# josiahbjorgaard/mca-paper

Measured on AMD Instinct MI355X. Metric: training samples/sec (fwd+bwd+opt), CMU 4-modality MCA, higher is better.
Workload: dtype bf16; 1 GPU; synthetic CMU 4-modality (MCA fcl), N=2538 D=512 L=5 H=8 F=88, lengths=full, p_drop=0.0; per_gpu_batch=32, global_batch=32, parallelism=dp1, inputs=device-resident, same batch every step, finite_checks=on (device flag, polled), attention_operands=bf16, attention_backward=bf16 one-pass, launch=hipGraph replay (one launch per step), collectives=none

## Files before the change

### include/mca_hip.h

```cpp
#ifndef MCA_HIP_H
#define MCA_HIP_H
#include <stdint.h>

#ifdef __cplusplus
extern "C" {
#endif

typedef void* mca_stream_t;

#define MCA_OK 0
#define MCA_E_BADARG (-1)
#define MCA_E_ALIGN (-2)
#define MCA_E_UNSUPPORTED (-3)
#define MCA_E_LAUNCH (-4)

const char* mca_version(void);

int mca_gemm_nt(const uint16_t* A, int64_t lda, const uint16_t* B, int64_t ldb,
                void* C, int64_t ldc, int out_bf16,
                const float* bias, const float* residual, int64_t ldres, int64_t res_period,
                int64_t M, int64_t N, int64_t K, mca_stream_t stream);

int mca_gemm_nt_lnres(const uint16_t* A, int64_t lda, const uint16_t* B, int64_t ldb, float* C, int64_t ldc,
                      const float* x, int64_t ldx, const float* mean, const float* rstd, const float* gamma,
                      int64_t M, int64_t N, int64_t K, mca_stream_t stream);

int mca_gemm_nt_geglu_bwd(const uint16_t* A, int64_t lda, const uint16_t* B, int64_t ldb, const uint16_t* h,
                          uint16_t* dh, int64_t ldh, int64_t ip, int64_t M, int64_t K, mca_stream_t stream);

int mca_gemm_nt_geglu_fwd(const uint16_t* A, int64_t lda, const uint16_t* W1, int64_t ldb, uint16_t* h, int64_t ldh,
                          uint16_t* g, int64_t ldg, int64_t ip, int64_t M, int64_t K, mca_stream_t stream);

int mca_gemm_tn_acc(const uint16_t* A, int64_t lda, const uint16_t* B, int64_t ldb,
                    float* C, int64_t ldc, int64_t R, int64_t N, int64_t K, mca_stream_t stream);

#define MCA_TN_MAX_GROUP 8
typedef struct mca_tn_desc {
  const uint16_t* A; int64_t lda;
  const uint16_t* B; int64_t ldb;
  float* C; int64_t ldc;
  int64_t N, K;
} mca_tn_desc;
int mca_gemm_tn_acc_group(const mca_tn_desc* d, int n, int64_t R, mca_stream_t stream);

int mca_layernorm_fwd(const float* x, int64_t ldx, const float* gamma, const float* beta,
                      const uint8_t* rowmask, const float* add, int64_t period,
                      float* y, int64_t ldy, int64_t y_bstride,
                      uint16_t* y_bf16, int64_t ld_bf16, int cols_pad,
                      float* mean, float* rstd, int64_t rows, int cols, float eps, mca_stream_t stream);

int mca_layernorm_bwd(const float* dy, int64_t ldy, int64_t y_bstride, int64_t period,
                      const float* x, int64_t ldx, const float* gamma,
                      const float* mean, const float* rstd, const uint8_t* rowmask,
                      float* dx, int64_t lddx, uint16_t* dx_bf16, int64_t ld_bf16,
                      float* dgamma, float* dbeta, float* dxsum, int64_t rows, int cols, mca_stream_t stream);

int mca_geglu_fwd(const uint16_t* h, uint16_t* g, int64_t rows, int ip, mca_stream_t stream);
// ... 163 lines not shown
```

### mca-paper_amd/csrc/gemm.hip

```cpp
#include "common.h"

#define g_knob mca_knobs

#define BM 128
#define BN 128
#define BK 64

static int num_cus() {
  static int n = 0;
  if (!n) {
    int dev = 0;
    if (hipGetDevice(&dev) != hipSuccess || hipDeviceGetAttribute(&n, hipDeviceAttributeMultiprocessorCount, dev) != hipSuccess || n <= 0) n = 256;
  }
  return n;
}

#define PS_PANELS 4
__device__ __forceinline__ void ps_tile_decode(int tile, int tiles_m, int tiles_n, int flat, int& tm, int& tn) {
  if (flat == 1) { tm = tile / tiles_n; tn = tile % tiles_n; return; }
  const int P = flat > 1 ? flat : PS_PANELS;
  const int per_group = P * tiles_n;
  const int g = tile / per_group;
  const int gh = (g + 1) * P <= tiles_m ? P : tiles_m - g * P;
  const int rem = tile - g * per_group;
// ... 790 lines not shown
        u16* cp = C + (int64_t)m * ldc + nw + 8 * (lane & 15);
        if (m < M) PS_GSTORE(cp, o[u]);
      }
      if (GEGLU) {
        asm volatile("s_waitcnt lgkmcnt(0)\n\ts_barrier" ::: "memory");
        const unsigned sa = lds_base + 3u * (unsigned)(P2_STAGE * 2) + (unsigned)(wave & ~1) * 8192u, sg = sa + 8192u;
        u32x4v av[4], gv[4];
#pragma unroll
        for (int u = 0; u < 4; u++) {
          const int row = 16 * wn + (lane >> 4) + 4 * u, ch = lane & 15;
          NT_DSREAD(av[u], sa + (unsigned)(row * 256 + ((ch ^ (row & 15)) << 4)));
          NT_DSREAD(gv[u], sg + (unsigned)(row * 256 + ((ch ^ (row & 15)) << 4)));
        }
        asm volatile("s_waitcnt lgkmcnt(0)" ::: "memory");
#pragma unroll
        for (int u = 0; u < 4; u++) {
          const int m = m0 + wm * 64 + i * 32 + 16 * wn + (lane >> 4) + 4 * u;
          u32x4v gg;
#pragma unroll
          for (int e = 0; e < 4; e++) {
            const float a0 = __uint_as_float(av[u][e] << 16), a1 = __uint_as_float(av[u][e] & 0xffff0000u);
            const float g0 = __uint_as_float(gv[u][e] << 16), g1 = __uint_as_float(gv[u][e] & 0xffff0000u);
            float ge0, ge1, unused;
            gelu_pair(g0, ge0, unused); gelu_pair(g1, ge1, unused);
            gg[e] = pack2bf(a0 * ge0, a1 * ge1);
          }
          u16* gp = G + (int64_t)m * ldg + tn * 128 + 8 * (lane & 15);
          if (m < M) PS_GSTORE(gp, gg);
        }
        if (i == 0) asm volatile("s_barrier" ::: "memory");
      }
    }
    if (edge) ps_wait_vm<0>();
    first = false;
    v = vn;
  }
}

extern "C" int mca_gemm_nt(const uint16_t* A, int64_t lda, const uint16_t* B, int64_t ldb, void* C, int64_t ldc,
                           int out_bf16, const float* bias, const float* residual, int64_t ldres,
                           int64_t res_period, int64_t M, int64_t N, int64_t K, mca_stream_t stream) {
  if (!A || !B || !C || M <= 0 || N <= 0 || K <= 0) return MCA_E_BADARG;
  if (K % 64 || lda % 8 || ldb % 8 || (uintptr_t)A % 16 || (uintptr_t)B % 16) return MCA_E_ALIGN;
  if (lda < K || ldb < K || ldc < N) return MCA_E_BADARG;
  if (M > (1LL << 30) || N > (1LL << 30)) return MCA_E_UNSUPPORTED;
  const int tiles_m = (int)((M + BM - 1) / BM), tiles_n = (int)((N + BN - 1) / BN);
  const int nwg = tiles_m * tiles_n;
  const int res = !residual ? 0 : (res_period > 0 ? 2 : 1);
  const bool big = M >= 2048 && g_knob[1] != 1;
  const int nwg2 = (int)((M + BM2 - 1) / BM2) * tiles_n;
#define NT_LAUNCH_G(OB, RS)                                                                                              \
  hipLaunchKernelGGL((gemm_nt_glds_kernel<OB, RS, 64, 0>), dim3(nwg), dim3(256), 0, as_stream(stream), A, lda, B, ldb, C,   \
                     ldc, bias, residual, ldres, res_period, (int)M, (int)N, (int)K, tiles_n, nwg)
#define NT_LAUNCH_256(OB, RS, PFV)                                                                                          \
  do {                                                                                                                   \
    static bool attr_dev[64] = {false}; bool& attr = *mca_dev_flag(attr_dev);                                                                                            \
    if (!attr) {                                                                                                         \
      if (hipFuncSetAttribute(reinterpret_cast<const void*>(gemm_nt_256_kernel<OB, RS, PFV, 0>),                            \
                              hipFuncAttributeMaxDynamicSharedMemorySize, NT256_LDS_BYTES) != hipSuccess)                \
        return MCA_E_LAUNCH;                                                                                             \
      attr = true;                                                                                                       \
    }                                                                                                                    \
    hipLaunchKernelGGL((gemm_nt_256_kernel<OB, RS, PFV, 0>), dim3(nwg2), dim3(512), NT256_LDS_BYTES, as_stream(stream), A, lda, \
                       B, ldb, C, ldc, bias, residual, ldres, res_period, (int)M, (int)N, (int)K, tiles_n, nwg2);        \
  } while (0)
#define NT_PICK_PF(OB, RS) do { if (big) NT_LAUNCH_256(OB, RS, 0); else NT_LAUNCH_G(OB, RS); } while (0)
// ... 31 lines not shown
    else if (res == 0) { if (bias) NT_LAUNCH_PS(1, true); else NT_LAUNCH_PS(1, false); }
    else { if (bias) NT_LAUNCH_PS(2, true); else NT_LAUNCH_PS(2, false); }
    return launch_status();
  }
  const bool pf = big && !out_bf16 && res == 1 && N % BN == 0 && K >= 512 && ldres % 4 == 0 && ldc % 4 == 0 &&
                  (uintptr_t)residual % 16 == 0 && (uintptr_t)C % 16 == 0 && (!bias || (uintptr_t)bias % 4 == 0) && g_knob[4] != 1;
  if (pf) { NT_LAUNCH_256(false, 1, 1); return launch_status(); }
  if (out_bf16) { if (res == 0) NT_PICK_PF(true, 0); else if (res == 1) NT_PICK_PF(true, 1); else NT_PICK_PF(true, 2); }
  else { if (res == 0) NT_PICK_PF(false, 0); else if (res == 1) NT_PICK_PF(false, 1); else NT_PICK_PF(false, 2); }
  return launch_status();
}


extern "C" int mca_gemm_nt_lnres(const uint16_t* A, int64_t lda, const uint16_t* B, int64_t ldb, float* C, int64_t ldc,
                                 const float* x, int64_t ldx, const float* mean, const float* rstd, const float* gamma,
                                 int64_t M, int64_t N, int64_t K, mca_stream_t stream) {
  if (!A || !B || !C || !x || !mean || !rstd || !gamma || M <= 0 || N <= 0 || K <= 0) return MCA_E_BADARG;
  if (K % 64 || lda % 8 || ldb % 8 || ldc % 4 || ldx % 4 || (uintptr_t)A % 16 || (uintptr_t)B % 16 || (uintptr_t)C % 16 ||
      (uintptr_t)x % 16 || (uintptr_t)gamma % 16)
    return MCA_E_ALIGN;
  if (lda < K || ldb < K || ldc < N || ldx < N) return MCA_E_BADARG;
  if (M < 2048 || M > (1LL << 30) || N % BN || K < 512) return MCA_E_UNSUPPORTED;
  const int tiles_n = (int)(N / BN);
  const int nwg2 = (int)((M + BM2 - 1) / BM2) * tiles_n;
  static bool attr_dev[64] = {false}; bool& attr = *mca_dev_flag(attr_dev);
  if (!attr) {
    if (hipFuncSetAttribute(reinterpret_cast<const void*>(gemm_nt_256_kernel<false, 1, 1, 2>), hipFuncAttributeMaxDynamicSharedMemorySize,
                            NT256LN_LDS_BYTES) != hipSuccess)
      return MCA_E_LAUNCH;
    attr = true;
  }
  hipLaunchKernelGGL((gemm_nt_256_kernel<false, 1, 1, 2>), dim3(nwg2), dim3(512), NT256LN_LDS_BYTES, as_stream(stream), A, lda, B, ldb,
                     (void*)C, ldc, (const float*)nullptr, x, ldx, (int64_t)0, (int)M, (int)N, (int)K, tiles_n, nwg2, mean, rstd, gamma);
  return launch_status();
}

extern "C" int mca_gemm_nt_geglu_bwd(const uint16_t* A, int64_t lda, const uint16_t* B, int64_t ldb, const uint16_t* h,
                                     uint16_t* dh, int64_t ldh, int64_t ip, int64_t M, int64_t K, mca_stream_t stream) {
  if (!A || !B || !h || !dh || M <= 0 || ip <= 0 || K <= 0) return MCA_E_BADARG;
  if (K % 64 || lda % 8 || ldb % 8 || ldh % 8 || ip % 8 || (uintptr_t)A % 16 || (uintptr_t)B % 16 || (uintptr_t)h % 16 || (uintptr_t)dh % 16)
    return MCA_E_ALIGN;
  if (lda < K || ldb < K || ldh < 2 * ip) return MCA_E_BADARG;
  if (M > (1LL << 30)) return MCA_E_UNSUPPORTED;
  const int64_t N = ip;
  const int tiles_n = (int)((N + BN - 1) / BN);
  const float* hres = reinterpret_cast<const float*>(h);
  void* C = dh;
  if (M >= 40960 && g_knob[1] != 1) {
    const int nwg2 = (int)((M + BM2 - 1) / BM2) * tiles_n;
    static bool attr_dev[64] = {false}; bool& attr = *mca_dev_flag(attr_dev);
    if (!attr) {
      if (hipFuncSetAttribute(reinterpret_cast<const void*>(gemm_nt_256_kernel<true, 0, 0, 1>), hipFuncAttributeMaxDynamicSharedMemorySize,
                              NT256_LDS_BYTES) != hipSuccess ||
          hipFuncSetAttribute(reinterpret_cast<const void*>(gemm_nt_persist_kernel<3, false>), hipFuncAttributeMaxDynamicSharedMemorySize,
                              NTPS_LDS_BYTES) != hipSuccess)
        return MCA_E_LAUNCH;
      attr = true;
    }
    if (g_knob[7] != 1 && N % BN == 0 && K >= 320) {
      const int grid = nwg2 < num_cus() ? nwg2 : num_cus();
      hipLaunchKernelGGL((gemm_nt_persist_kernel<3, false>), dim3(grid), dim3(512), NTPS_LDS_BYTES, as_stream(stream), A, lda, B, ldb, C, ldh,
                         nullptr, hres, ldh, (int)M, (int)N, (int)K, tiles_n, nwg2, g_knob[0]);
    } else
      hipLaunchKernelGGL((gemm_nt_256_kernel<true, 0, 0, 1>), dim3(nwg2), dim3(512), NT256_LDS_BYTES, as_stream(stream), A, lda, B, ldb, C,
                         ldh, nullptr, hres, ldh, 0, (int)M, (int)N, (int)K, tiles_n, nwg2);
  } else {
// ... 673 lines not shown
```

### mca-paper_amd/engine.py

```python
from __future__ import annotations

import os

import ctypes as C
import math
from typing import Callable, Dict, List, Optional

import numpy as np
import torch

from . import attention, hip
from .attention import AttnGrads, AttnOperands, _OnePassSched, _Sched, _dev
from .encoders import EmbeddedSequenceEncoder, TabularEncoder
from .hip import AttnBwd1Args, AttnBwd2Args, AttnFp8BwdOperands, AttnFp8Operands, AttnFwdArgs, LossTerm, call, ptr, stream_ptr

LN_EPS = 1e-5
FWD_BQ, FWD_BK = 128, 64
BWD_BQ = 64


def _pad_to(x: int, m: int) -> int:
    return (x + m - 1) // m * m


def debug_options() -> dict:
    opts = {"overlap_wgrad": None, "group_wgrad": True, "mask_mfma": True, "dkv_keys": 128, "lazy_softmax": True,
            "onepass": None}
    for item in filter(None, os.environ.get("MCA_DEBUG", "").split(",")):
        k, _, v = item.partition("=")
        k = k.strip()
        if k not in opts:
            raise ValueError(f"MCA_DEBUG: unknown switch '{k}' (known: {sorted(opts)})")
        opts[k] = int(v) if k == "dkv_keys" else (v.strip() not in ("0", "", "false"))
    return opts


class FusionEngine:
    def __init__(self, model):
        self.model = model
        p0 = next(model.parameters())
        self.eao = model.attn_pool is None
        if p0.device.type != "cuda":
            raise hip.MCAHipError("the MCA step runs only on a HIP device: move the model to cuda first "
                                  "(there is no CPU fallback)")
        hip.lib()
        self.device = p0.device
        self.D, self.H, self.L = model.dim, model.heads, model.depth
        st = model.structure
        self.st = st
        self.N, self.R, self.F, self.M = st.n_tokens, st.n_return, st.num_fusion_tokens, st.n_modalities
        if self.D != self.H * 64:
            raise NotImplementedError("native path needs dim == heads * 64")
        self.I = model.layers[0].ff.inner_dim if self.L else int(self.D * 4 * 2 / 3)
        self.Ip = _pad_to(self.I, 64)
        self.scale = model.dim_head ** -0.5
        self.q_scale = self.scale * 1.4426950408889634
        self.attn_flags = hip.ATTN_Q_PRESCALED
        self.attn_dtype = "bf16"
        self.dbg = debug_options()
        if self.dbg["lazy_softmax"]:
            self.attn_flags |= hip.ATTN_LAZY_REFERENCE
        self.nk_pad = _pad_to(self.N, 256)
        self.mask_mfma = int(self.st.kgroup.max()) <= 14 and self.dbg["mask_mfma"]
        self._flatten_parameters()
        self._build_static()
        self._alloc_weights()
        self._ws: Dict[int, dict] = {}
        self._weights_version = -1
        self.grad_bucket_hook: Optional[Callable[[int, int], None]] = None
        self.gather_hook: Optional[Callable] = None
        self.check_finite = True
        self.finite_flag = torch.zeros(1, dtype=torch.int32, device=self.device)
        self._flag_host = torch.zeros(1, dtype=torch.int32).pin_memory()
        self._flag_event: Optional[torch.cuda.Event] = None
        self.fuse_geglu_bwd = True
        self._mod_shifts = torch.arange(len(model.modality_types), dtype=torch.int32, device=self.device)
        self.fuse_ln_residual = True
        self.overlap_wgrad = self.dbg["overlap_wgrad"]
        self.group_wgrad = self.dbg["group_wgrad"]

    def _flatten_parameters(self):
        m = self.model
        order: List[torch.nn.Parameter] = []
        marks: List[int] = []
        order += [m.loss.loss_fn.logit_scale]
        pool_kv_late = not self.eao and self.L > 0
        if not self.eao:
            order += [m.return_tokens, m.attn_pool.to_out.weight, m.attn_pool.to_q.weight]
            if not pool_kv_late:
                order += [m.attn_pool.to_kv.weight]
        order += [m.norm.gamma]
        marks.append(len(order))
        if pool_kv_late:
            order += [m.attn_pool.to_kv.weight]
        for i in reversed(range(self.L)):
            ly = m.layers[i]
            order += [ly.ff.feedforward[2].weight, ly.ff.feedforward[0].weight, ly.attn.to_out.weight,
                      ly.attn.to_q.weight, ly.attn.to_kv.weight, ly.norm.gamma]
            marks.append(len(order))
        if not self.eao:
            order.append(m.fusion_tokens)
        for name in m.modality_types:
            order += list(m.encoders[name].parameters())
        marks.append(len(order))
        seen = {id(p) for p in order}
        for p in m.parameters():
            if id(p) not in seen:
                order.append(p)
        marks[-1] = len(order)
        offs, n = [], 0
# ... 207 lines not shown
        ws["dpool_b"], ws["dop"], ws["dqp32"], ws["dqp_sum"], ws["dqp_b"] = bf(b * R, D), bf(b * R, D), f32(b * R, D), f32(R, D), bf(R, D)
        ws["dkvp"], ws["drt"] = (None if self.eao else bf(T, 2 * D)), f32(R, D)
        sc = self.sched_onepass
        if sc is not None:
            rc = f32(b, H, sc.n_qt + 1, 2, 64)
            rc[:, :, :, 0] = float("-inf"); rc[:, :, :, 1] = 0.0
            ws["rowc"] = rc
            ws["dq_acc"] = f32(b * H * self.backward_plan(ws, b, N).split * (sc.n_qt + 1) * 4096)
            ws["q_hm"] = torch.zeros((b * H * N + 64) * 64, dtype=torch.bfloat16, device=dev)
            ws["do_hm"] = torch.zeros((b * H * N + 64) * 64, dtype=torch.bfloat16, device=dev)
        ws["enc"] = {}
        for mi, name in enumerate(self.model.modality_types):
            enc = self.model.encoders[name]
            n = self.st.token_dims[mi]
            rows = b * n
            if isinstance(enc, EmbeddedSequenceEncoder):
                kp = self.we[name]["kp"]
                ws["enc"][name] = dict(xin_b=bf(rows, kp), m0=f32(rows), r0=f32(rows), y=f32(rows, D), m2=f32(rows), r2=f32(rows),
                                       dy=f32(rows, D), dy_b=bf(rows, D), dxin=f32(rows, kp), mask=u8(rows))
            elif isinstance(enc, TabularEncoder):
                ws["enc"][name] = dict(h1_b=bf(rows, D), y=f32(rows, D), m2=f32(rows), r2=f32(rows), dy=f32(rows, D),
                                       dy_b=bf(rows, D), dh1=f32(rows, D), mask=u8(rows))
        ws["side"], ws["side_events"] = torch.cuda.Stream(device=dev), []
        self._ws[b] = ws
        return ws

    @staticmethod
    def gemm_nt(A, B, C, M, N, K, bias=None, residual=None, res_period=0):
        if hip.PROFILE is not None:
            hip.set_tag(f"{M}x{N}x{K}{'' if C.dtype == torch.bfloat16 else ' f32'}{' +res' if residual is not None else ''}")
        call("mca_gemm_nt", ptr(A), A.stride(0), ptr(B), B.stride(0), ptr(C), C.stride(0), int(C.dtype == torch.bfloat16),
             ptr(bias), ptr(residual), residual.stride(0) if residual is not None else 0, res_period, M, N, K, stream_ptr(),
             flops=2.0 * M * N * K)
        if hip.PROFILE is not None:
            hip.set_tag("")

    @staticmethod
    def gemm_tn_acc(A, B, Cgrad, R, N, K):
        call("mca_gemm_tn_acc", ptr(A), A.stride(0), ptr(B), B.stride(0), ptr(Cgrad), Cgrad.stride(0), R, N, K, stream_ptr(),
             flops=2.0 * R * N * K)

    @staticmethod
    def gemm_tn_acc_group(members, R):
        arr = (hip.TnDesc * len(members))()
        fl = 0.0
        for d, (A, B, Cg, N, K) in zip(arr, members):
            d.A, d.lda, d.B, d.ldb, d.C, d.ldc, d.N, d.K = ptr(A), A.stride(0), ptr(B), B.stride(0), ptr(Cg), Cg.stride(0), N, K
            fl += 2.0 * R * N * K
        call("mca_gemm_tn_acc_group", C.byref(arr), len(members), R, stream_ptr(), flops=fl)

    @staticmethod
    def ln_fwd(x, gamma, rows, cols, mean, rstd, beta=None, rowmask=None, add=None, period=0, y=None, ldy=0, y_bstride=0,
               y_bf16=None, cols_pad=0):
        call("mca_layernorm_fwd", ptr(x), x.stride(0), ptr(gamma), ptr(beta), ptr(rowmask), ptr(add), period,
             ptr(y), ldy, y_bstride, ptr(y_bf16), y_bf16.stride(0) if y_bf16 is not None else 0, cols_pad,
             ptr(mean), ptr(rstd), rows, cols, LN_EPS, stream_ptr())

    @staticmethod
    def ln_bwd(dy, ldy, x, gamma, mean, rstd, rows, cols, dgamma, dbeta=None, rowmask=None, dx=None, dx_bf16=None,
               y_bstride=0, period=0, dxsum=None):
        call("mca_layernorm_bwd", ptr(dy), ldy, y_bstride, period, ptr(x), x.stride(0), ptr(gamma), ptr(mean), ptr(rstd),
             ptr(rowmask), ptr(dx), dx.stride(0) if dx is not None else 0, ptr(dx_bf16),
             dx_bf16.stride(0) if dx_bf16 is not None else 0, ptr(dgamma), ptr(dbeta), ptr(dxsum), rows, cols, stream_ptr())

    def layer_attention(self, ws, i):
        D, N, a = self.D, self.N, ws["layers"][i]
# ... 318 lines not shown
        pool_kv = (ws["dkvp"], ws["t_b"], G(ap.to_kv.weight), 2 * D, D)
        if not (self.L > 0 and self.group_wgrad and T >= 4096):
            on_side(lambda pk=pool_kv: tn(pk[0], pk[1], pk[2], T, 2 * D, D))
            pool_kv = None
        dx, dx_other = ws["dxa"], ws["dxb"]
        self.gemm_nt(ws["dkvp"], self.wp["kvT"], dx, T, D, 2 * D)
        top = ws["layers"][self.L - 1]["dxo_b"] if self.L else ws["dx_b"]
        self.ln_bwd(dx, D, ws["x"][self.L], m.norm.gamma, ws["mf"], ws["rf"], T, D, G(m.norm.gamma), dx=dx_other, dx_bf16=top)
        dx, dx_other = dx_other, dx
        on_side(lambda: bucket_ready(0))
        self._backward_layers_and_encoders(ws, dx, dx_other, bucket_ready, on_side, extra_top=pool_kv)

    def _backward_part_eao(self, ws, dpool, bucket_ready, on_side):
        m, D, N, R, b, T = self.model, self.D, self.N, self.R, ws["b"], ws["T"]
        dx, dx_other = ws["dxa"], ws["dxb"]
        call("mca_segment_mean_bwd", ptr(dpool), ptr(ws["padding"]), ptr(self.kgroup), ptr(ws["seg_counts"]), R, ptr(dx), b, N, D,
             stream_ptr())
        top = ws["layers"][self.L - 1]["dxo_b"] if self.L else ws["dx_b"]
        self.ln_bwd(dx, D, ws["x"][self.L], m.norm.gamma, ws["mf"], ws["rf"], T, D, self.grad_of(m.norm.gamma), dx=dx_other, dx_bf16=top)
        dx, dx_other = dx_other, dx
        on_side(lambda: bucket_ready(0))
        self._backward_layers_and_encoders(ws, dx, dx_other, bucket_ready, on_side)

    def _backward_layers_and_encoders(self, ws, dx, dx_other, bucket_ready, on_side, extra_top=None):
        m, D, N, H, Ip, I, R, b, T = self.model, self.D, self.N, self.H, self.Ip, self.I, self.R, ws["b"], ws["T"]
        G = self.grad_of
        tn = self.gemm_tn_acc
        for bi, i in enumerate(reversed(range(self.L))):
            ly, w, a = m.layers[i], self.wl[i], ws["layers"][i]
            g = ly.norm.gamma
            dxo, dx1, dh, dqkv = a["dxo_b"], a["dx1_b"], a["dh"], a["dqkv"]
            below = ws["layers"][i - 1]["dxo_b"] if i > 0 else ws["dx_b"]
            grouped = self.group_wgrad and T >= 4096
            if not grouped:
                on_side(lambda dxo=dxo, a=a, ly=ly: tn(dxo, a["g"], G(ly.ff.feedforward[2].weight), T, D, I))
            if self.fuse_geglu_bwd:
                call("mca_gemm_nt_geglu_bwd", ptr(dxo), D, ptr(w["w2T"]), D, ptr(a["h"]), ptr(dh), 2 * Ip, Ip, T, D,
                     stream_ptr(), flops=2.0 * T * Ip * D)
            else:
                self.gemm_nt(dxo, w["w2T"], ws["dg"], T, Ip, D)
                call("mca_geglu_bwd", ptr(ws["dg"]), ptr(a["h"]), ptr(dh), T, Ip, stream_ptr())
            gw1 = G(ly.ff.feedforward[0].weight)
            if not grouped:
                on_side(lambda dh=dh, a=a, gw1=gw1: (tn(dh, a["x1n_b"], gw1, T, I, D), tn(dh[:, Ip:], a["x1n_b"], gw1[I:], T, I, D)))
            self.gemm_nt(dh, w["w1T"], dx_other, T, D, 2 * Ip, residual=dx)
            self.ln_bwd(dx_other, D, a["x1"], g, a["m2"], a["r2"], T, D, G(g), dx=dx, dx_bf16=dx1)
            if not grouped:
                on_side(lambda dx1=dx1, a=a, ly=ly: tn(dx1, a["o"], G(ly.attn.to_out.weight), T, D, D))
            self.gemm_nt(dx1, w["oT"], ws["do"], T, D, D)
            self.attn_backward(*self.layer_attention(ws, i), ws)
            gq = G(ly.attn.to_q.weight)
            assert G(ly.attn.to_kv.weight).data_ptr() == gq.data_ptr() + D * D * 4
            if grouped:
                gw2, gwo = G(ly.ff.feedforward[2].weight), G(ly.attn.to_out.weight)
                extra = [extra_top] if (bi == 0 and extra_top is not None) else []
                on_side(lambda dqkv=dqkv, dh=dh, dxo=dxo, dx1=dx1, a=a, gq=gq, gw1=gw1, gw2=gw2, gwo=gwo, extra=extra: self.gemm_tn_acc_group(
                    [(dqkv, a["xn_b"], gq, 3 * D, D), (dh, a["x1n_b"], gw1, I, D), (dh[:, Ip:], a["x1n_b"], gw1[I:], I, D),
                     (dxo, a["g"], gw2, D, I), (dx1, a["o"], gwo, D, D)] + extra, T))
            else:
                on_side(lambda dqkv=dqkv, a=a, gq=gq: tn(dqkv, a["xn_b"], gq, T, 3 * D, D))
            self.gemm_nt(dqkv, w["qkvT"], dx_other, T, D, 3 * D, residual=dx)
            self.ln_bwd(dx_other, D, ws["x"][i], g, a["m1"], a["r1"], T, D, G(g), dx=dx, dx_bf16=below)
            on_side(lambda bi=bi: bucket_ready(bi + 1))
        if self.eao:
            for src, dst, n in self.st.copies:
                call("mca_rows_copy_add", dx.data_ptr() + dst * D * 4, N * D, dx.data_ptr() + src * D * 4, N * D, n, D, b, 1, stream_ptr())
        if self.F:
            call("mca_reduce_rows", dx.data_ptr() + (N - self.F) * D * 4, D, N * D, self.F, ptr(G(m.fusion_tokens)), D,
                 b * self.F, D, stream_ptr())
        for mi, name in enumerate(m.modality_types):
            enc = m.encoders[name]
            n, off = self.st.token_dims[mi], self.offsets[mi]
            rows = b * n
            if isinstance(enc, EmbeddedSequenceEncoder):
                e, te = ws["enc"][name], enc.token_encoder
                kp = self.we[name]["kp"]
                self.ln_bwd(dx[off:], D, e["y"], te[2].weight, e["m2"], e["r2"], rows, D, G(te[2].weight), dbeta=G(te[2].bias),
                            rowmask=e["mask"], dx=e["dy"], dx_bf16=e["dy_b"], y_bstride=N * D, period=n, dxsum=G(te[1].bias))
                on_side(lambda e=e, te=te, rows=rows, enc=enc: tn(e["dy_b"], e["xin_b"], G(te[1].weight), rows, D, enc.input_size))
                self.gemm_nt(e["dy_b"], self.we[name]["wT"], e["dxin"], rows, kp, D)
                t2 = e["tokens"].view(rows, enc.input_size)
                self.ln_bwd(e["dxin"], kp, t2, te[0].weight, e["m0"], e["r0"], rows, enc.input_size, G(te[0].weight),
                            dbeta=G(te[0].bias), rowmask=e["mask"])
            elif isinstance(enc, TabularEncoder):
                self._backward_tabular(name, enc, ws, mi, dx)
            else:
                toks = ws["foreign"][name]
                if toks.requires_grad:
                    for p in enc.parameters():
                        p.grad = G(p)
                    torch.autograd.backward(toks, dx.view(b, N, D)[:, off:off + n].to(toks.dtype))
        on_side(lambda: bucket_ready(len(self.bucket_bounds) - 1))

    def _backward_tabular(self, name, enc, ws, mi, dx):
        D, N, b = self.D, self.N, ws["b"]
# ... 164 lines not shown
```

### mca-paper_amd/hip.py

```python
from __future__ import annotations

import ctypes as C
import os
from typing import Optional

import torch

_HERE = os.path.dirname(os.path.abspath(__file__))
LIB_PATH = os.environ.get("MCA_HIP_LIB") or os.path.join(_HERE, "libmca_hip.so")

_ERR = {-1: "bad argument", -2: "misaligned pointer / leading dimension", -3: "unsupported size", -4: "launch failed"}


class MCAHipError(RuntimeError):
    pass


class LossTerm(C.Structure):
    _fields_ = [("slot_a", C.c_int32), ("slot_b", C.c_int32), ("and_bits", C.c_uint32), ("or_bits", C.c_uint32)]


class CastDesc(C.Structure):
    _fields_ = [("src", C.c_void_p), ("dst", C.c_void_p), ("lds", C.c_int64), ("rows", C.c_int64), ("cols", C.c_int64),
                ("ldd", C.c_int64), ("rows_pad", C.c_int64), ("cols_pad", C.c_int64), ("transpose", C.c_int32), ("scale", C.c_float)]
# ... 66 lines not shown
    ]


class AttnBwd1Args(C.Structure):
    _fields_ = [
        ("q", C.c_void_p), ("q_bstride", C.c_int64), ("q_ld", C.c_int64),
        ("k", C.c_void_p), ("v", C.c_void_p), ("kv_bstride", C.c_int64), ("kv_ld", C.c_int64),
        ("d_o", C.c_void_p), ("o_bstride", C.c_int64), ("o_ld", C.c_int64),
        ("q_hstride", C.c_int64), ("o_hstride", C.c_int64),
        ("rowc", C.c_void_p), ("dvmean", C.c_void_p),
        ("dq", C.c_void_p), ("dq_bstride", C.c_int64), ("dq_ld", C.c_int64),
        ("dk", C.c_void_p), ("dv", C.c_void_p), ("dkv_bstride", C.c_int64), ("dkv_ld", C.c_int64),
        ("dq_acc", C.c_void_p),
        ("keyinfo", C.c_void_p), ("ktile_flags", C.c_void_p), ("khot", C.c_void_p), ("qblk", C.c_void_p),
        ("qt_desc", C.c_void_p), ("kb_desc", C.c_void_p), ("kb_qt", C.c_void_p), ("visit", C.c_void_p),
        ("n_qtiles", C.c_int), ("n_kblocks", C.c_int), ("max_list", C.c_int), ("n_entries", C.c_int),
        ("batch", C.c_int), ("heads", C.c_int), ("n", C.c_int), ("nk_pad", C.c_int), ("n_ktiles64", C.c_int),
        ("scale", C.c_float), ("flags", C.c_int), ("split", C.c_int),
    ]


_P, _I64, _I, _F = C.c_void_p, C.c_int64, C.c_int, C.c_float

SIGNATURES = {
    "mca_version": (C.c_char_p, []),
    "mca_flag_to_host": (_I, [_P, _P, _P]),
    "mca_build_keyhot": (_I, [_P, _P, _I, _I, _P]),
    "mca_rows_copy_add": (_I, [_P, _I64, _P, _I64, _I64, _I, _I, _I, _P]),
    "mca_segment_mean_fwd": (_I, [_P, _P, _P, _I, _P, _P, _I, _I, _I, _P]),
    "mca_segment_mean_bwd": (_I, [_P, _P, _P, _P, _I, _P, _I, _I, _I, _P]),
    "mca_gemm_nt": (_I, [_P, _I64, _P, _I64, _P, _I64, _I, _P, _P, _I64, _I64, _I64, _I64, _I64, _P]),
    "mca_gemm_nt_geglu_bwd": (_I, [_P, _I64, _P, _I64, _P, _P, _I64, _I64, _I64, _I64, _P]),
    "mca_gemm_nt_lnres": (_I, [_P, _I64, _P, _I64, _P, _I64, _P, _I64, _P, _P, _P, _I64, _I64, _I64, _P]),
    "mca_gemm_nt_geglu_fwd": (_I, [_P, _I64, _P, _I64, _P, _I64, _P, _I64, _I64, _I64, _I64, _P]),
    "mca_gemm_tn_acc": (_I, [_P, _I64, _P, _I64, _P, _I64, _I64, _I64, _I64, _P]),
    "mca_gemm_tn_acc_group": (_I, [_P, _I, _I64, _P]),
    "mca_layernorm_fwd": (_I, [_P, _I64, _P, _P, _P, _P, _I64, _P, _I64, _I64, _P, _I64, _I, _P, _P, _I64, _I, _F, _P]),
    "mca_layernorm_bwd": (_I, [_P, _I64, _I64, _I64, _P, _I64, _P, _P, _P, _P, _P, _I64, _P, _I64, _P, _P, _P, _I64, _I, _P]),
    "mca_geglu_fwd": (_I, [_P, _P, _I64, _I, _P]),
    "mca_geglu_bwd": (_I, [_P, _P, _P, _I64, _I, _P]),
    "mca_cast_pad_bf16": (_I, [_P, _I64, _I64, _I64, _P, _I64, _I64, _I64, _I, _P]),
    "mca_cast_pad_bf16_multi": (_I, [_P, _I, _P]),
    "mca_f32_to_bf16": (_I, [_P, _I64, _P, _I64, _I64, _I64, _F, _P]),
    "mca_bcast_rows": (_I, [_P, _I64, _P, _I64, _I64, _I64, _I64, _I, _P]),
    "mca_reduce_rows": (_I, [_P, _I64, _I64, _I64, _P, _I64, _I64, _I, _P]),
    "mca_embedding_renorm": (_I, [_P, _I64, _I, _F, _P]),
    "mca_tab_value_fwd": (_I, [_P, _P, _P, _P, _P, _I64, _I, _F, _F, _P]),
    "mca_tab_value_bwd": (_I, [_P, _I64, _P, _P, _P, _P, _I64, _I, _F, _P]),
    "mca_pack_masks": (_I, [_P, _P, _P, _P]),
    "mca_build_keyinfo": (_I, [_P, _P, _P, _P, _I, _I, _I, _P]),
    "mca_attn_vmean": (_I, [_P, _I64, _I64, _P, _I, _I, _I, _P]),
    "mca_attn_vmean_if_needed": (_I, [_P, _I64, _I64, _P, _I, _I, _I, _P, _I, _P]),
    "mca_attn_fwd": (_I, [C.POINTER(AttnFwdArgs), _P]),
    "mca_attn_quant_mxfp8": (_I, [_P, _I64, _I64, _P, _P, _I64, _I64, C.POINTER(AttnFp8Operands), _I, _I, _I, _P]),
    "mca_attn_fwd_fp8": (_I, [C.POINTER(AttnFwdArgs), C.POINTER(AttnFp8Operands), _P]),
    "mca_attn_bwd_prep": (_I, [_P, _P, _I64, _I64, _P, _P, _P, _I, _I, _I, _I, _P]),
    "mca_attn_bwd_onepass": (_I, [C.POINTER(AttnBwd1Args), _P]),
    "mca_attn_bwd_prep_onepass": (_I, [_P, _P, _I64, _I64, _P, _P, _P, _P, _I, _I, _I, _I, _P, _I64, _I64, _P, _P, _P]),
    "mca_attn_bwd_dq": (_I, [C.POINTER(AttnBwd2Args), _P]),
    "mca_attn_bwd_dkv": (_I, [C.POINTER(AttnBwd2Args), _P]),
    "mca_attn_quant_bwd_mxfp8": (_I, [_P, _I64, _I64, _P, _P, _I64, _I64, _P, _I64, _I64, C.POINTER(AttnFp8BwdOperands), _I, _I, _I, _I, _P]),
    "mca_attn_bwd_dq_fp8": (_I, [C.POINTER(AttnBwd2Args), C.POINTER(AttnFp8BwdOperands), _P]),
    "mca_attn_bwd_dkv_fp8": (_I, [C.POINTER(AttnBwd2Args), C.POINTER(AttnFp8BwdOperands), _P]),
    "mca_contrastive_workspace_bytes": (_I64, [_I, _I]),
    "mca_contrastive_fwd_bwd": (_I, [_P, _P, _P, _I, _P, _I, _I, _I, _I, _I, _P, _P, _P, _P, _P, _P]),
    "mca_grad_sqnorm": (_I, [_P, _I64, _P, _P]),
# ... 102 lines not shown


def profile_enable(flag: bool):
    global _PROFILE_ON
    _PROFILE_ON = bool(flag)


def set_tag(tag: str):
    global _TAG
    _TAG = tag


def profile_start(names):
    global PROFILE
    PROFILE = {"names": set(names), "records": {}}


def profile_collect():
    torch.cuda.synchronize()
    tot = PROFILE.setdefault("totals", {})
    for key, recs in PROFILE["records"].items():
        n, ms, fl = tot.get(key, (0, 0.0, 0.0))
        tot[key] = (n + len(recs), ms + sum(s.elapsed_time(e) for s, e, _ in recs), fl + sum(f for _, _, f in recs))
    PROFILE["records"] = {}


def profile_stop():
    global PROFILE
    profile_collect()
    prof, PROFILE = PROFILE, None
    return prof["totals"]


def call(name: str, *args, flops: float = 0.0):
    if PROFILE is not None and _PROFILE_ON and name in PROFILE["names"]:
        s, e = torch.cuda.Event(enable_timing=True), torch.cuda.Event(enable_timing=True)
        s.record()
        check(getattr(lib(), name)(*args), name)
        e.record()
        PROFILE["records"].setdefault(name + ("/" + _TAG if _TAG else ""), []).append((s, e, flops))
        return
    check(getattr(lib(), name)(*args), name)
```

Measured before the change: 1694 samples/s.

## Fuse backward GEMM with residual add and LayerNorm backward in row-owning kernel

Adds a persistent kernel in which each workgroup owns full 128-row by 512-column output tiles of the input-gradient GEMM. In the epilogue it adds the residual gradient, computes the LayerNorm backward row reductions through LDS, and writes dx in fp32 and bf16, with dgamma accumulated through LDS then global atomics. It replaces the separate GEMM-with-residual plus ln_bwd pair for both LN sites in each layer's backward pass, removing the fp32 intermediate round trip and one launch per site. In exchange the grid is limited to one row-tile per workgroup with N fixed at 512, so parallelism drops for the GEMM. dgamma is summed with float atomics, so its accumulation order is no longer fixed.

Result: no change. 1694 samples/s, median of 2 (-0.0%).

```diff
diff --git a/include/mca_hip.h b/include/mca_hip.h
--- a/include/mca_hip.h
+++ b/include/mca_hip.h
@@ -23,6 +23,11 @@
 
 int mca_gemm_nt_lnres(const uint16_t* A, int64_t lda, const uint16_t* B, int64_t ldb, float* C, int64_t ldc,
                       const float* x, int64_t ldx, const float* mean, const float* rstd, const float* gamma,
+                      int64_t M, int64_t N, int64_t K, mca_stream_t stream);
+
+int mca_gemm_nt_lnbwd(const uint16_t* A, int64_t lda, const uint16_t* B, int64_t ldb, const float* res, int64_t ldres,
+                      const float* x, int64_t ldx, const float* gamma, const float* mean, const float* rstd,
+                      float* dx, int64_t lddx, uint16_t* dx_bf16, int64_t ld_bf16, float* dgamma,
                       int64_t M, int64_t N, int64_t K, mca_stream_t stream);
 
 int mca_gemm_nt_geglu_bwd(const uint16_t* A, int64_t lda, const uint16_t* B, int64_t ldb, const uint16_t* h,
diff --git a/mca-paper_amd/csrc/gemm.hip b/mca-paper_amd/csrc/gemm.hip
--- a/mca-paper_amd/csrc/gemm.hip
+++ b/mca-paper_amd/csrc/gemm.hip
@@ -846,6 +846,263 @@
       }
     }
     if (edge) ps_wait_vm<0>();
+    first = false;
+    v = vn;
+  }
+}
+
+#define RF_BM 128
+#define RF_STAGE ((RF_BM + 512) * 32)
+#define RF_SCR_OFF (3 * RF_STAGE * 2)
+#define RF_DGS_OFF (RF_SCR_OFF + 8 * 4096)
+#define RF_LDS_BYTES (RF_DGS_OFF + 2048)
+__global__ __launch_bounds__(512) void gemm_nt_rowfused_lnbwd_kernel(
+    const u16* __restrict__ A, int64_t lda, const u16* __restrict__ B, int ldb, const float* res, int ldres,
+    const float* __restrict__ x, int ldx, const float* __restrict__ gamma, const float* __restrict__ mean,
+    const float* __restrict__ rstd, float* dx, int lddx, u16* __restrict__ dxb, int ld_bf16,
+    float* __restrict__ dgamma, int M, int K, int ntiles) {
+  extern __shared__ __attribute__((aligned(16))) u16 lds2[];
+  const int tid = threadIdx.x, lane = tid & 63, wave = __builtin_amdgcn_readfirstlane(tid >> 6);
+  const int wm = wave >> 2, wn = wave & 3;
+  const int nkt = K / 32;
+  const unsigned lds_base = (unsigned)(uintptr_t)(__attribute__((address_space(3))) const u16*)lds2;
+  char* lds_bytes = reinterpret_cast<char*>(lds2);
+  float* scr = reinterpret_cast<float*>(lds_bytes + RF_SCR_OFF + wave * 4096);
+  float* red = reinterpret_cast<float*>(lds_bytes + 2 * RF_STAGE * 2);
+  float* dgs = reinterpret_cast<float*>(lds_bytes + RF_DGS_OFF);
+
+  int v = blockIdx.x;
+  if (v >= ntiles) return;
+  dgs[tid] = 0.f;
+  bool first = true;
+  while (v < ntiles) {
+    const int m0 = v * RF_BM;
+    int lk = lane;
+    asm volatile("" : "+v"(lk));
+    unsigned fa_addr[2], fb_addr[4];
+    {
+      const int l31 = lk & 31, lh = lk >> 5;
+#pragma unroll
+      for (int i = 0; i < 2; i++) { const int r = wm * 64 + i * 32 + l31; fa_addr[i] = lds_base + (unsigned)(r * 64 + ((lh ^ gl_sw<32>(r)) << 4)); }
+#pragma unroll
+      for (int j = 0; j < 4; j++) { const int r = wn * 128 + j * 32 + l31; fb_addr[j] = lds_base + (unsigned)(RF_BM * 64) + (unsigned)(r * 64 + ((lh ^ gl_sw<32>(r)) << 4)); }
+    }
+    const u16* ga;
+    const u16* gb[4];
+#pragma unroll
+    for (int i = 0; i < 4; i++) {
+      const int p = (i * 8 + wave) * 64 + lk, r = p >> 2, c = (p & 3) ^ gl_sw<32>(r);
+      gb[i] = B + (unsigned)(r * ldb + c * 8);
+    }
+    auto tile_ptrs = [&](int tile) {
+      const int p = wave * 64 + lk, r = p >> 2, c = (p & 3) ^ gl_sw<32>(r);
+      int ra = tile * RF_BM + r; if (ra > M - 1) ra = M - 1;
+      ga = A + (int64_t)ra * lda + c * 8;
+    };
+    auto stage = [&](int k0, int st) {
+      u16* base = lds2 + st * RF_STAGE;
+      __builtin_amdgcn_global_load_lds((const __attribute__((address_space(1))) void*)(ga + k0),
+                                       (__attribute__((address_space(3))) void*)(base + wave * 512), 16, 0, 0);
+#pragma unroll
+      for (int i = 0; i < 4; i++)
+        __builtin_amdgcn_global_load_lds((const __attribute__((address_space(1))) void*)(gb[i] + k0),
+                                         (__attribute__((address_space(3))) void*)(base + RF_BM * 32 + (i * 8 + wave) * 512), 16, 0, 0);
+    };
+    tile_ptrs(v);
+    if (first) { stage(0, 0); stage(32, 1); }
+    f32x16 acc[2][4];
+#pragma unroll
+    for (int i = 0; i < 2; i++)
+#pragma unroll
+      for (int j = 0; j < 4; j++)
+#pragma unroll
+        for (int r = 0; r < 16; r++) acc[i][j][r] = 0.f;
+#define RF_SB __builtin_amdgcn_sched_barrier(0);
+#define RF_RA(KS, I) NT_DSREAD(fa[KS][I], (fa_addr[I] + so) ^ (32u * (KS))); RF_SB
+#define RF_RB(KS, J) NT_DSREAD(fb[KS][J], (fb_addr[J] + so) ^ (32u * (KS))); RF_SB
+#define RF_MM(KS, I, J) acc[I][J] = __builtin_amdgcn_mfma_f32_32x32x16_bf16(*reinterpret_cast<const bf16x8*>(&fb[KS][J]), \
+                                                                            *reinterpret_cast<const bf16x8*>(&fa[KS][I]), acc[I][J], 0, 0, 0); RF_SB
+    int st = 0;
+    for (int kt = 0; kt < nkt; kt++) {
+      if (first || kt >= 2) { if (kt + 1 < nkt) ps_wait_vm<5>(); else ps_wait_vm<0>(); }
+      __builtin_amdgcn_s_barrier();
+      if (kt + 2 < nkt) { int s2 = st + 2; if (s2 >= 3) s2 -= 3; stage((kt + 2) * 32, s2); }
+      const unsigned so = (unsigned)st * (unsigned)(RF_STAGE * 2);
+      u32x4v fa[2][2], fb[2][4];
+      RF_SB
+      RF_RA(0, 0) RF_RB(0, 0) RF_RB(0, 1) RF_RB(0, 2) RF_RB(0, 3) RF_RA(0, 1)
+      RF_RA(1, 0) RF_RB(1, 0) RF_RB(1, 1) RF_RB(1, 2) RF_RB(1, 3) RF_RA(1, 1)
+      asm volatile("s_waitcnt lgkmcnt(6)" ::: "memory"); RF_SB
+      RF_MM(0, 0, 0) RF_MM(0, 0, 1) RF_MM(0, 0, 2) RF_MM(0, 0, 3) RF_MM(0, 1, 0) RF_MM(0, 1, 1) RF_MM(0, 1, 2) RF_MM(0, 1, 3)
+      asm volatile("s_waitcnt lgkmcnt(0)" ::: "memory"); RF_SB
+      RF_MM(1, 0, 0) RF_MM(1, 0, 1) RF_MM(1, 0, 2) RF_MM(1, 0, 3) RF_MM(1, 1, 0) RF_MM(1, 1, 1) RF_MM(1, 1, 2) RF_MM(1, 1, 3)
+      st = st == 2 ? 0 : st + 1;
+    }
+#undef RF_RA
+#undef RF_RB
+#undef RF_MM
+    __builtin_amdgcn_s_barrier();
+    const int vn = v + gridDim.x;
+    if (vn < ntiles) {
+      tile_ptrs(vn);
+      stage(0, 0); stage(32, 1);
+    }
+    asm volatile("" ::: "memory"); RF_SB
+    const int rows_left = M - m0;
+    const char* res_t = reinterpret_cast<const char*>(res + (int64_t)m0 * ldres);
+    const char* x_t = reinterpret_cast<const char*>(x + (int64_t)m0 * ldx);
+    char* dx_t = reinterpret_cast<char*>(dx + (int64_t)m0 * lddx);
+    char* dxb_t = reinterpret_cast<char*>(dxb + (int64_t)m0 * ld_bf16);
+#pragma unroll
+    for (int i = 0; i < 2; i++) {
+      f32x4 dyv[4][4];
+      {
+        int le = lane;
+        asm volatile("" : "+v"(le));
+        const int e31 = le & 31, eh = le >> 5, lr = le >> 3, lc = le & 7;
+        const int colw = wn * 128 + 4 * lc;
+        const int rloc = wm * 64 + i * 32 + lr;
+        bool live[4]; int mr[4]; float mu[4], rs[4];
+#pragma unroll
+        for (int u = 0; u < 4; u++) {
+          live[u] = rloc + 8 * u < rows_left;
+          mr[u] = live[u] ? rloc + 8 * u : rows_left - 1;
+          mu[u] = mean[m0 + mr[u]]; rs[u] = rstd[m0 + mr[u]];
+        }
+        float s1[4] = {0.f, 0.f, 0.f, 0.f}, s2[4] = {0.f, 0.f, 0.f, 0.f};
+        f32x4 rv[2][2], xv[2][2];
+        auto fetch = [&](int s) {
+#pragma unroll
+          for (int w = 0; w < 2; w++) {
+            const int u = 2 * (s & 1) + w;
+            rv[s & 1][w] = __builtin_nontemporal_load(reinterpret_cast<const f32x4*>(res_t + (unsigned)(mr[u] * ldres + colw + 32 * (s >> 1)) * 4u));
+            xv[s & 1][w] = *reinterpret_cast<const f32x4*>(x_t + (unsigned)(mr[u] * ldx + colw + 32 * (s >> 1)) * 4u);
+          }
+        };
+        fetch(0);
+        f32x4 gm, dgj;
+#pragma unroll
+        for (int s = 0; s < 8; s++) {
+          const int j = s >> 1, h = s & 1;
+          if (h == 0) {
+            gm = *reinterpret_cast<const f32x4*>(gamma + colw + 32 * j);
+            dgj = f32x4{0.f, 0.f, 0.f, 0.f};
+#pragma unroll
+            for (int q = 0; q < 4; q++)
+              *reinterpret_cast<f32x4*>(scr + e31 * 32 + (((2 * q + eh) ^ (e31 & 7)) << 2)) =
+                  f32x4{acc[i][j][4 * q], acc[i][j][4 * q + 1], acc[i][j][4 * q + 2], acc[i][j][4 * q + 3]};
+            __builtin_amdgcn_wave_barrier();
+          }
+          f32x4 t[2];
+#pragma unroll
+          for (int w = 0; w < 2; w++) { const int row = lr + 8 * (2 * h + w); t[w] = *reinterpret_cast<const f32x4*>(scr + row * 32 + ((lc ^ (row & 7)) << 2)); }
+          __builtin_amdgcn_wave_barrier();
+          if (i == 0 && s == 0) ps_wait_vm<0>();
+          if (s < 7) fetch(s + 1);
+          RF_SB
+#pragma unroll
+          for (int w = 0; w < 2; w++) {
+            const int u = 2 * h + w;
+#pragma unroll
+            for (int e = 0; e < 4; e++) {
+              const float d = t[w][e] + rv[s & 1][w][e];
+              const float xh_ = (xv[s & 1][w][e] - mu[u]) * rs[u];
+              const float g_ = d * gm[e];
+              dgj[e] += live[u] ? d * xh_ : 0.f;
+              s1[u] += g_; s2[u] += g_ * xh_;
+              dyv[j][u][e] = d;
+            }
+            asm volatile("" : "+v"(s1[u]), "+v"(s2[u]));
+            RF_SB
+          }
+          if (h == 1) {
+#pragma unroll
+            for (int o = 8; o < 64; o <<= 1) {
+              f32x4 tq;
+#pragma unroll
+              for (int e = 0; e < 4; e++) tq[e] = __shfl_xor(dgj[e], o, WAVE);
+              dgj += tq;
+            }
+            if (lr == 0) {
+#pragma unroll
+              for (int e = 0; e < 4; e++) if (dgj[e] != 0.f) atomicAdd(dgs + colw + 32 * j + e, dgj[e]);
+            }
+          }
+          RF_SB
+        }
+#pragma unroll
+        for (int o = 1; o < 8; o <<= 1) {
+          float t1[4], t2[4];
+#pragma unroll
+          for (int u = 0; u < 4; u++) { t1[u] = __shfl_xor(s1[u], o, WAVE); t2[u] = __shfl_xor(s2[u], o, WAVE); }
+#pragma unroll
+          for (int u = 0; u < 4; u++) { s1[u] += t1[u]; s2[u] += t2[u]; }
+        }
+#pragma unroll
+        for (int u = 0; u < 4; u++) {
+          if (lc == 0) { float* rp = red + ((i * RF_BM + rloc + 8 * u) * 4 + wn) * 2; rp[0] = s1[u]; rp[1] = s2[u]; }
+        }
+      }
+      asm volatile("s_waitcnt lgkmcnt(0)\n\ts_barrier" ::: "memory");
+      {
+        int le = lane;
+        asm volatile("" : "+v"(le));
+        const int lr = le >> 3, lc = le & 7;
+        const bool odd = le & 1;
+        const int colw = wn * 128 + 4 * lc;
+        const int rloc = wm * 64 + i * 32 + lr;
+        bool live[4]; int mr[4];
+        float c1[4], c2[4], mu[4], rs[4];
+#pragma unroll
+        for (int u = 0; u < 4; u++) {
+          live[u] = rloc + 8 * u < rows_left;
+          mr[u] = live[u] ? rloc + 8 * u : rows_left - 1;
+          mu[u] = mean[m0 + mr[u]]; rs[u] = rstd[m0 + mr[u]];
+          const float* rp = red + (i * RF_BM + rloc + 8 * u) * 8;
+          const f32x4 p0 = *reinterpret_cast<const f32x4*>(rp), p1 = *reinterpret_cast<const f32x4*>(rp + 4);
+          c1[u] = ((p0[0] + p0[2]) + (p1[0] + p1[2])) * (1.f / 512.f);
+          c2[u] = ((p0[1] + p0[3]) + (p1[1] + p1[3])) * (1.f / 512.f);
+        }
+        f32x4 xv[2][2];
+        auto fetch = [&](int s) {
+#pragma unroll
+          for (int w = 0; w < 2; w++)
+            xv[s & 1][w] = __builtin_nontemporal_load(reinterpret_cast<const f32x4*>(x_t + (unsigned)(mr[2 * (s & 1) + w] * ldx + colw + 32 * (s >> 1)) * 4u));
+        };
+        fetch(0);
+        f32x4 gm;
+#pragma unroll
+        for (int s = 0; s < 8; s++) {
+          const int j = s >> 1, h = s & 1;
+          if (h == 0) gm = *reinterpret_cast<const f32x4*>(gamma + colw + 32 * j);
+          if (s < 7) fetch(s + 1);
+          uint32_t pk[2][2];
+#pragma unroll
+          for (int w = 0; w < 2; w++) {
+            const int u = 2 * h + w;
+            f32x4 o;
+#pragma unroll
+            for (int e = 0; e < 4; e++) o[e] = rs[u] * (dyv[j][u][e] * gm[e] - c1[u] - ((xv[s & 1][w][e] - mu[u]) * rs[u]) * c2[u]);
+            if (live[u]) __builtin_nontemporal_store(o, reinterpret_cast<f32x4*>(dx_t + (unsigned)(mr[u] * lddx + colw + 32 * j) * 4u));
+            pk[w][0] = pack2bf(o[0], o[1]); pk[w][1] = pack2bf(o[2], o[3]);
+            RF_SB
+          }
+          const uint32_t own0 = odd ? pk[1][0] : pk[0][0], own1 = odd ? pk[1][1] : pk[0][1];
+          const uint32_t snd0 = odd ? pk[0][0] : pk[1][0], snd1 = odd ? pk[0][1] : pk[1][1];
+          const uint32_t rcv0 = (uint32_t)__shfl_xor((int)snd0, 1, WAVE), rcv1 = (uint32_t)__shfl_xor((int)snd1, 1, WAVE);
+          uint4 w4;
+          w4.x = odd ? rcv0 : own0; w4.y = odd ? rcv1 : own1; w4.z = odd ? own0 : rcv0; w4.w = odd ? own1 : rcv1;
+          const int rowb = rloc + 16 * h + (odd ? 8 : 0);
+          if (rowb < rows_left) *reinterpret_cast<uint4*>(dxb_t + (unsigned)(rowb * ld_bf16 + colw - (odd ? 4 : 0) + 32 * j) * 2u) = w4;
+          RF_SB
+        }
+      }
+    }
+    {
+      const float sm = dgs[tid];
+      if (sm != 0.f) { atomicAdd(dgamma + tid, sm); dgs[tid] = 0.f; }
+    }
+#undef RF_SB
     first = false;
     v = vn;
   }
@@ -943,6 +1200,31 @@
   }
   hipLaunchKernelGGL((gemm_nt_256_kernel<false, 1, 1, 2>), dim3(nwg2), dim3(512), NT256LN_LDS_BYTES, as_stream(stream), A, lda, B, ldb,
                      (void*)C, ldc, (const float*)nullptr, x, ldx, (int64_t)0, (int)M, (int)N, (int)K, tiles_n, nwg2, mean, rstd, gamma);
+  return launch_status();
+}
+
+extern "C" int mca_gemm_nt_lnbwd(const uint16_t* A, int64_t lda, const uint16_t* B, int64_t ldb, const float* res, int64_t ldres,
+                                 const float* x, int64_t ldx, const float* gamma, const float* mean, const float* rstd,
+                                 float* dx, int64_t lddx, uint16_t* dx_bf16, int64_t ld_bf16, float* dgamma,
+                                 int64_t M, int64_t N, int64_t K, mca_stream_t stream) {
+  if (!A || !B || !res || !x || !gamma || !mean || !rstd || !dx || !dx_bf16 || !dgamma || M <= 0 || N <= 0 || K <= 0) return MCA_E_BADARG;
+  if (N != 512 || K % 64 || K < 128 || M > (1LL << 30)) return MCA_E_UNSUPPORTED;
+  if (lda % 8 || ldb % 8 || ldres % 4 || ldx % 4 || lddx % 4 || ld_bf16 % 8 || (uintptr_t)A % 16 || (uintptr_t)B % 16 ||
+      (uintptr_t)res % 16 || (uintptr_t)x % 16 || (uintptr_t)gamma % 16 || (uintptr_t)dx % 16 || (uintptr_t)dx_bf16 % 16)
+    return MCA_E_ALIGN;
+  if (lda < K || ldb < K || ldres < N || ldx < N || lddx < N || ld_bf16 < N) return MCA_E_BADARG;
+  if (ldb > (1 << 20) || ldres > (1 << 20) || ldx > (1 << 20) || lddx > (1 << 20) || ld_bf16 > (1 << 20)) return MCA_E_UNSUPPORTED;
+  static bool attr_dev[64] = {false}; bool& attr = *mca_dev_flag(attr_dev);
+  if (!attr) {
+    if (hipFuncSetAttribute(reinterpret_cast<const void*>(gemm_nt_rowfused_lnbwd_kernel), hipFuncAttributeMaxDynamicSharedMemorySize,
+                            RF_LDS_BYTES) != hipSuccess)
+      return MCA_E_LAUNCH;
+    attr = true;
+  }
+  const int ntiles = (int)((M + RF_BM - 1) / RF_BM);
+  const int grid = ntiles < num_cus() ? ntiles : num_cus();
+  hipLaunchKernelGGL(gemm_nt_rowfused_lnbwd_kernel, dim3(grid), dim3(512), RF_LDS_BYTES, as_stream(stream), A, lda, B, (int)ldb, res, (int)ldres,
+                     x, (int)ldx, gamma, mean, rstd, dx, (int)lddx, dx_bf16, (int)ld_bf16, dgamma, (int)M, (int)K, ntiles);
   return launch_status();
 }
 
diff --git a/mca-paper_amd/engine.py b/mca-paper_amd/engine.py
--- a/mca-paper_amd/engine.py
+++ b/mca-paper_amd/engine.py
@@ -25,7 +25,8 @@
 
 def debug_options() -> dict:
     opts = {"overlap_wgrad": None, "group_wgrad": True, "mask_mfma": True, "dkv_keys": 128, "lazy_softmax": True,
-            "onepass": None}
+            "onepass": None,
+            "rowfused": True}
     for item in filter(None, os.environ.get("MCA_DEBUG", "").split(",")):
         k, _, v = item.partition("=")
         k = k.strip()
@@ -76,6 +77,7 @@
         self.fuse_geglu_bwd = True
         self._mod_shifts = torch.arange(len(model.modality_types), dtype=torch.int32, device=self.device)
         self.fuse_ln_residual = True
+        self.rowfused = self.dbg["rowfused"]
         self.overlap_wgrad = self.dbg["overlap_wgrad"]
         self.group_wgrad = self.dbg["group_wgrad"]
 
@@ -349,6 +351,16 @@
         call("mca_gemm_nt", ptr(A), A.stride(0), ptr(B), B.stride(0), ptr(C), C.stride(0), int(C.dtype == torch.bfloat16),
              ptr(bias), ptr(residual), residual.stride(0) if residual is not None else 0, res_period, M, N, K, stream_ptr(),
              flops=2.0 * M * N * K)
+        if hip.PROFILE is not None:
+            hip.set_tag("")
+
+    @staticmethod
+    def gemm_nt_lnbwd(A, B, dx, x, gamma, mean, rstd, dx_bf16, dgamma, M, N, K):
+        if hip.PROFILE is not None:
+            hip.set_tag(f"{M}x{N}x{K} f32 +lnbwd")
+        call("mca_gemm_nt_lnbwd", ptr(A), A.stride(0), ptr(B), B.stride(0), ptr(dx), dx.stride(0), ptr(x), x.stride(0), ptr(gamma),
+             ptr(mean), ptr(rstd), ptr(dx), dx.stride(0), ptr(dx_bf16), dx_bf16.stride(0), ptr(dgamma), M, N, K, stream_ptr(),
+             flops=2.0 * M * N * K, timed_as="mca_gemm_nt")
         if hip.PROFILE is not None:
             hip.set_tag("")
 
@@ -733,6 +745,7 @@
             dxo, dx1, dh, dqkv = a["dxo_b"], a["dx1_b"], a["dh"], a["dqkv"]
             below = ws["layers"][i - 1]["dxo_b"] if i > 0 else ws["dx_b"]
             grouped = self.group_wgrad and T >= 4096
+            rowfused = self.rowfused and self.fuse_ln_residual and T >= 2048 and D == 512 and Ip >= 512
             if not grouped:
                 on_side(lambda dxo=dxo, a=a, ly=ly: tn(dxo, a["g"], G(ly.ff.feedforward[2].weight), T, D, I))
             if self.fuse_geglu_bwd:
@@ -744,8 +757,11 @@
             gw1 = G(ly.ff.feedforward[0].weight)
             if not grouped:
                 on_side(lambda dh=dh, a=a, gw1=gw1: (tn(dh, a["x1n_b"], gw1, T, I, D), tn(dh[:, Ip:], a["x1n_b"], gw1[I:], T, I, D)))
-            self.gemm_nt(dh, w["w1T"], dx_other, T, D, 2 * Ip, residual=dx)
-            self.ln_bwd(dx_other, D, a["x1"], g, a["m2"], a["r2"], T, D, G(g), dx=dx, dx_bf16=dx1)
+            if rowfused:
+                self.gemm_nt_lnbwd(dh, w["w1T"], dx, a["x1"], g, a["m2"], a["r2"], dx1, G(g), T, D, 2 * Ip)
+            else:
+                self.gemm_nt(dh, w["w1T"], dx_other, T, D, 2 * Ip, residual=dx)
+                self.ln_bwd(dx_other, D, a["x1"], g, a["m2"], a["r2"], T, D, G(g), dx=dx, dx_bf16=dx1)
             if not grouped:
                 on_side(lambda dx1=dx1, a=a, ly=ly: tn(dx1, a["o"], G(ly.attn.to_out.weight), T, D, D))
             self.gemm_nt(dx1, w["oT"], ws["do"], T, D, D)
@@ -760,8 +776,11 @@
                      (dxo, a["g"], gw2, D, I), (dx1, a["o"], gwo, D, D)] + extra, T))
             else:
                 on_side(lambda dqkv=dqkv, a=a, gq=gq: tn(dqkv, a["xn_b"], gq, T, 3 * D, D))
-            self.gemm_nt(dqkv, w["qkvT"], dx_other, T, D, 3 * D, residual=dx)
-            self.ln_bwd(dx_other, D, ws["x"][i], g, a["m1"], a["r1"], T, D, G(g), dx=dx, dx_bf16=below)
+            if rowfused:
+                self.gemm_nt_lnbwd(dqkv, w["qkvT"], dx, ws["x"][i], g, a["m1"], a["r1"], below, G(g), T, D, 3 * D)
+            else:
+                self.gemm_nt(dqkv, w["qkvT"], dx_other, T, D, 3 * D, residual=dx)
+                self.ln_bwd(dx_other, D, ws["x"][i], g, a["m1"], a["r1"], T, D, G(g), dx=dx, dx_bf16=below)
             on_side(lambda bi=bi: bucket_ready(bi + 1))
         if self.eao:
             for src, dst, n in self.st.copies:
diff --git a/mca-paper_amd/hip.py b/mca-paper_amd/hip.py
--- a/mca-paper_amd/hip.py
+++ b/mca-paper_amd/hip.py
@@ -122,6 +122,7 @@
     "mca_gemm_nt": (_I, [_P, _I64, _P, _I64, _P, _I64, _I, _P, _P, _I64, _I64, _I64, _I64, _I64, _P]),
     "mca_gemm_nt_geglu_bwd": (_I, [_P, _I64, _P, _I64, _P, _P, _I64, _I64, _I64, _I64, _P]),
     "mca_gemm_nt_lnres": (_I, [_P, _I64, _P, _I64, _P, _I64, _P, _I64, _P, _P, _P, _I64, _I64, _I64, _P]),
+    "mca_gemm_nt_lnbwd": (_I, [_P, _I64, _P, _I64, _P, _I64, _P, _I64, _P, _P, _P, _P, _I64, _P, _I64, _P, _I64, _I64, _I64, _P]),
     "mca_gemm_nt_geglu_fwd": (_I, [_P, _I64, _P, _I64, _P, _I64, _P, _I64, _I64, _I64, _I64, _P]),
     "mca_gemm_tn_acc": (_I, [_P, _I64, _P, _I64, _P, _I64, _I64, _I64, _I64, _P]),
     "mca_gemm_tn_acc_group": (_I, [_P, _I, _I64, _P]),
@@ -290,12 +291,13 @@
     return prof["totals"]
 
 
-def call(name: str, *args, flops: float = 0.0):
-    if PROFILE is not None and _PROFILE_ON and name in PROFILE["names"]:
+def call(name: str, *args, flops: float = 0.0, timed_as: Optional[str] = None):
+    key = timed_as or name
+    if PROFILE is not None and _PROFILE_ON and key in PROFILE["names"]:
         s, e = torch.cuda.Event(enable_timing=True), torch.cuda.Event(enable_timing=True)
         s.record()
         check(getattr(lib(), name)(*args), name)
         e.record()
-        PROFILE["records"].setdefault(name + ("/" + _TAG if _TAG else ""), []).append((s, e, flops))
+        PROFILE["records"].setdefault(key + ("/" + _TAG if _TAG else ""), []).append((s, e, flops))
         return
     check(getattr(lib(), name)(*args), name)
```
